# sea-sky-web/Vision-based-Spatio-Temporal-Analysis

Measured on AMD Instinct MI355X. Metric: multi-cam frames/sec (7-cam→480×1440 BEV), higher is better.
Workload: dtype f32; 1 GPU; 7-cam 1080x1920 -> resnet50(stride-8 features)+proj C=64 -> IPM warp -> mean -> 480x1440 BEV (BASELINE configs[1]); cameras=7, cameras_per_gpu=7, channels=64, bev_memory_format=NCHW, parallelism=frame-sharded x1 (no collective)

## Files before the change

### vision-based-spatio-temporal-analysis_amd/csrc/bev_conv_x6.hip

```cpp
#include <hip/hip_runtime.h>
#include <stdint.h>

#include <type_traits>

#include "../../include/bev_mi355x.h"
#include "bev_act.h"

namespace {

typedef __bf16 bf16x8 __attribute__((ext_vector_type(8)));
typedef __bf16 bf16x4 __attribute__((ext_vector_type(4)));
typedef float f32x16 __attribute__((ext_vector_type(16)));
typedef float f32x4 __attribute__((ext_vector_type(4)));
typedef unsigned u32x4 __attribute__((ext_vector_type(4)));
typedef unsigned u32x2 __attribute__((ext_vector_type(2)));

#ifndef X6S_T_EPI
#define X6S_T_EPI 0
#endif
#ifndef X6S_ABLATE
#define X6S_ABLATE 0
#endif
constexpr int XBK = 16;
constexpr int XROW = 24;

__device__ __attribute__((aligned(16))) float g_xzero4[4] = {0.f, 0.f, 0.f, 0.f};

__host__ __device__ inline int64_t kpad_x(int K) { return (K + XBK - 1) / XBK * XBK; }
__host__ __device__ inline int64_t copad_x(int Co) { return (Co + 127) / 128 * 128; }

__device__ __forceinline__ void split3(float v, __bf16 &h, __bf16 &m, __bf16 &l) {
    h = (__bf16)v;
    const float r = v - (float)h;
    m = (__bf16)r;
    l = (__bf16)(r - (float)m);
}

__host__ __device__ inline int64_t frag_index(int n, int k, int p, int64_t S) {
    return (((int64_t)(n >> 5) * S + (k >> 4)) * 3 + p) * 512 + (((k >> 3) & 1) * 32 + (n & 31)) * 8 + (k & 7);
}

__global__ void k_pack_x6(const float *__restrict__ w, int Co, int Ci, int KH, int KW, int64_t Kp, int64_t Cop,
                          __bf16 *__restrict__ out) {
    const int64_t t = (int64_t)blockIdx.x * blockDim.x + threadIdx.x;
    if (t >= Kp * Cop) return;
    const int n = (int)(t / Kp);
    const int k = (int)(t % Kp);
    const int K = Ci * KH * KW;
    float v = 0.0f;
    if (n < Co && k < K) {
        const int ci = k % Ci, r = k / Ci, kx = r % KW, ky = r / KW;
        v = w[(((int64_t)n * Ci + ci) * KH + ky) * KW + kx];
    }
    __bf16 h, m, l;
    split3(v, h, m, l);
    const int64_t S = Kp / XBK;
    out[frag_index(n, k, 0, S)] = h;
    out[frag_index(n, k, 1, S)] = m;
    out[frag_index(n, k, 2, S)] = l;
}

struct ConvX {
    const float *__restrict__ x;
    const __bf16 *__restrict__ wp;
    const float *__restrict__ bias;
    const float *__restrict__ res;
    float *__restrict__ y;
    int N, H, W, Ci, Co, KH, KW, stride, pad, dil, Ho, Wo, act, ldy, Kp;
    int64_t M;
    const float *__restrict__ x2;
    int Ci2, H2, W2, stride2;
    const __bf16 *__restrict__ xs;
    __bf16 *__restrict__ ys;
    int64_t xps, yps;
    const __bf16 *__restrict__ wp2;
    const float *__restrict__ bias2;
    int Co2, act2;
    int nta = 0;
    const __bf16 *__restrict__ wp3 = nullptr;
    const float *__restrict__ bias3 = nullptr;
    __bf16 *__restrict__ ys3 = nullptr;
    float *__restrict__ y3 = nullptr;
    int Co3 = 0, act3 = 0;
};

__device__ __forceinline__ float act_x(float t, int act) {
    if (act == 2) return silu_hw(t);
    if (act == 1) return t > 0.0f ? t : 0.0f;
    return t;
}

template <int TN>
__host__ __device__ constexpr int x6_epi_bytes() { return 4 * 32 * (TN * 32 + 4) * 4; }

template <int TM, int TN>
__device__ __forceinline__ void x6_epilogue(const ConvX &a, float *lds, const f32x16 (&acc)[TM][TN], int wave,
                                            int lane, int wn, int wm, int64_t m0, int n0) {
    const int r32 = lane & 31, h = lane >> 5;
    constexpr int WC = TN * 32, ER = WC + 4;
    constexpr int C4 = WC / 4, RPI = 64 / C4, NQ = 32 / RPI;
    float *E = lds + wave * (32 * ER);
    const int c4 = lane % C4, rq = lane / C4;
    const int n = n0 + wn * WC + c4 * 4;
    const bool nvec = ((a.Co & 3) == 0) && ((a.ldy & 3) == 0) && (n + 3 < a.Co);
    float4 rv[NQ];
    auto res_load = [&](int i) {
        const int64_t mb = m0 + wm * TM * 32 + i * 32;
#pragma unroll
        for (int q = 0; q < NQ; ++q) {
            const int64_t m = mb + rq + RPI * q;
            rv[q] = make_float4(0.f, 0.f, 0.f, 0.f);
            if (a.res && m < a.M && nvec) rv[q] = *(const float4 *)(a.res + m * a.Co + n);
        }
    };
    res_load(0);
    __syncthreads();
    float4 bv = make_float4(0.f, 0.f, 0.f, 0.f);
    if (a.bias) {
        if (nvec) bv = *(const float4 *)(a.bias + n);
        else {
            bv.x = n < a.Co ? a.bias[n] : 0.f;
            bv.y = n + 1 < a.Co ? a.bias[n + 1] : 0.f;
            bv.z = n + 2 < a.Co ? a.bias[n + 2] : 0.f;
            bv.w = n + 3 < a.Co ? a.bias[n + 3] : 0.f;
        }
    }
#pragma unroll
    for (int i = 0; i < TM; ++i) {
#pragma unroll
        for (int j = 0; j < TN; ++j)
#pragma unroll
            for (int r = 0; r < 16; ++r) E[((r & 3) + 8 * (r >> 2) + 4 * h) * ER + j * 32 + r32] = acc[i][j][r];
        const int64_t mbase = m0 + wm * TM * 32 + i * 32;
        if (i > 0) res_load(i);
#pragma unroll
        for (int q = 0; q < NQ; ++q) {
            const int row = rq + RPI * q;
            const int64_t m = mbase + row;
            if (m >= a.M) continue;
            const float4 v = *(const float4 *)(E + row * ER + c4 * 4);
            float o[4] = {v.x + bv.x, v.y + bv.y, v.z + bv.z, v.w + bv.w};
            if (a.ys) {
                if (a.res) {
                    const float4 rr = rv[q];
                    o[0] += rr.x, o[1] += rr.y, o[2] += rr.z, o[3] += rr.w;
                }
                bf16x4 hv, mv, lv;
#pragma unroll
                for (int u = 0; u < 4; ++u) {
                    __bf16 h_, m_, l_;
                    split3(act_x(o[u], a.act), h_, m_, l_);
                    hv[u] = h_, mv[u] = m_, lv[u] = l_;
                }
                __bf16 *yp = a.ys + m * a.Co + n;
                if (n < a.Co) {
                    *(bf16x4 *)yp = hv;
                    *(bf16x4 *)(yp + a.yps) = mv;
                    *(bf16x4 *)(yp + 2 * a.yps) = lv;
                }
                continue;
            }
            float *yp = a.y + m * a.ldy + n;
            if (nvec) {
                if (a.res) {
                    o[0] += rv[q].x;
                    o[1] += rv[q].y;
                    o[2] += rv[q].z;
                    o[3] += rv[q].w;
                }
#pragma unroll
                for (int u = 0; u < 4; ++u) o[u] = act_x(o[u], a.act);
                *(float4 *)yp = make_float4(o[0], o[1], o[2], o[3]);
            } else {
#pragma unroll
                for (int u = 0; u < 4; ++u) {
                    if (n + u >= a.Co) break;
                    float t = o[u];
                    if (a.res) t += a.res[m * a.Co + n + u];
                    yp[u] = act_x(t, a.act);
                }
            }
        }
    }
}

template <int WM, int WN, int TM, int TN, bool DUAL>
__global__ __launch_bounds__(256, 2) void k_conv_x6(ConvX a) {
    constexpr int BM = WM * TM * 32, BN = WN * TN * 32;
    constexpr int APL = BM * XROW, BPL = BN * XROW;
    constexpr int STAGE = 3 * (APL + BPL);
    constexpr int AQ = BM / 64;
    constexpr int PB = ((BN * 6) % 256 == 0) ? 16 : 8;
    constexpr int PPR = 96 / PB;
    constexpr int BQ = BN * PPR / 256;
    static_assert(BN * PPR % 256 == 0, "B pieces per thread");
    typedef typename std::conditional<PB == 16, u32x4, u32x2>::type bpiece;
    constexpr int EPIB = x6_epi_bytes<TN>();
    constexpr int LDSB = (2 * STAGE * 2 > EPIB) ? 2 * STAGE * 2 : EPIB;
    static_assert(BM % 64 == 0, "A staging rows");
    __shared__ __attribute__((aligned(16))) unsigned char lds_raw[LDSB];
    __bf16 *lds = (__bf16 *)lds_raw;

    const int tid = threadIdx.x;
    const int lane = tid & 63, wave = __builtin_amdgcn_readfirstlane(tid >> 6);
    const int wm = wave / WN, wn = wave % WN;
    const int n_tiles = (a.Co + BN - 1) / BN;
    unsigned bid = blockIdx.x;
    {
        const unsigned nb = gridDim.x, q = nb / 8, r = nb % 8, xc = bid % 8;
        bid = (xc < r ? xc * (q + 1) : r * (q + 1) + (xc - r) * q) + bid / 8;
    }
    const int64_t m0 = (int64_t)(bid / n_tiles) * BM;
    const int n0 = (bid % n_tiles) * BN;

    const int aq = tid & 3;
    int64_t pb[AQ], p2[AQ];
    int iy0[AQ], ix0[AQ];
    bool rok[AQ];
#pragma unroll
    for (int q = 0; q < AQ; ++q) {
        const int64_t m = m0 + (tid >> 2) + 64 * q;
        rok[q] = m < a.M;
        const int64_t mm = rok[q] ? m : 0;
        const int ox = (int)(mm % a.Wo);
        const int64_t t = mm / a.Wo;
        const int oy = (int)(t % a.Ho);
        const int64_t n = t / a.Ho;
        if (DUAL) {
            pb[q] = mm * a.Ci + 4 * aq;
            p2[q] = ((n * a.H2 + (int64_t)oy * a.stride2) * a.W2 + (int64_t)ox * a.stride2) * a.Ci2 + 4 * aq;
            iy0[q] = ix0[q] = 0;
        } else {
            pb[q] = n * a.H * a.W * a.Ci + 4 * aq;
            p2[q] = 0;
            iy0[q] = oy * a.stride - a.pad;
            ix0[q] = ox * a.stride - a.pad;
        }
    }
    const int64_t bstep = 3 * 512;
    const __bf16 *brow[BQ];
    int bdst[BQ];
#pragma unroll
    for (int i = 0; i < BQ; ++i) {
        const int pc = tid + 256 * i;
        const int row = pc / PPR, byte = (pc % PPR) * PB;
        const int pl = byte / 32, hk = (byte % 32) / 16, sub = (byte % 16) / 2;
        brow[i] = a.wp + frag_index(n0 + row, 8 * hk, pl, a.Kp / XBK) + sub;
        bdst[i] = pl * BPL + row * XROW + 8 * hk + sub;
    }
    f32x16 acc[TM][TN];
#pragma unroll
    for (int i = 0; i < TM; ++i)
#pragma unroll
        for (int j = 0; j < TN; ++j) acc[i][j] = (f32x16){0};

    f32x4 va0[AQ], va1[AQ];
    bpiece vb0[BQ], vb1[BQ];
    int ky = 0, kx = 0, ci0 = 0, k0 = 0;
    int64_t kb = 0;
#define X6_GLOAD(VA, VB)                                                                                   \
    do {                                                                                                   \
        if (DUAL) {                                                                                        \
            const bool first = k0 < a.Ci;                                                                  \
            const float *src = first ? a.x + k0 : a.x2 + (k0 - a.Ci);                                      \
            _Pragma("unroll") for (int q = 0; q < AQ; ++q) VA[q] =                                         \
                *(const f32x4 *)(rok[q] ? src + (first ? pb[q] : p2[q]) : g_xzero4);                      \
// ... 23 lines not shown
        __bf16 *Bs = As + 3 * APL;                                                                         \
        _Pragma("unroll") for (int q = 0; q < AQ; ++q) {                                                   \
            bf16x4 hv, mv, lv;                                                                             \
            _Pragma("unroll") for (int e = 0; e < 4; ++e) {                                                \
                __bf16 h_, m_, l_;                                                                         \
                split3(VA[q][e], h_, m_, l_);                                                              \
                hv[e] = h_;                                                                                \
                mv[e] = m_;                                                                                \
                lv[e] = l_;                                                                                \
            }                                                                                              \
            __bf16 *d = As + ((tid >> 2) + 64 * q) * XROW + 4 * aq;                                        \
            *(bf16x4 *)d = hv;                                                                             \
            *(bf16x4 *)(d + APL) = mv;                                                                     \
            *(bf16x4 *)(d + 2 * APL) = lv;                                                                 \
        }                                                                                                  \
        _Pragma("unroll") for (int i = 0; i < BQ; ++i) *(bpiece *)(Bs + bdst[i]) = VB[i];                \
    } while (0)
    const int r32 = lane & 31, h = lane >> 5;
#define X6_MFMA(BUF)                                                                                       \
    do {                                                                                                   \
        const __bf16 *As = lds + (BUF) * STAGE;                                                            \
        const __bf16 *Bs = As + 3 * APL;                                                                   \
        bf16x8 fa[TM][3], fb[TN][3];                                                                       \
        _Pragma("unroll") for (int i = 0; i < TM; ++i)                                                     \
            _Pragma("unroll") for (int p = 0; p < 3; ++p)                                                  \
                fa[i][p] = *(const bf16x8 *)(As + p * APL + (wm * TM * 32 + i * 32 + r32) * XROW + 8 * h); \
        _Pragma("unroll") for (int j = 0; j < TN; ++j)                                                     \
            _Pragma("unroll") for (int p = 0; p < 3; ++p)                                                  \
                fb[j][p] = *(const bf16x8 *)(Bs + p * BPL + (wn * TN * 32 + j * 32 + r32) * XROW + 8 * h); \
        _Pragma("unroll") for (int i = 0; i < TM; ++i)                                                     \
            _Pragma("unroll") for (int j = 0; j < TN; ++j) {                                               \
                acc[i][j] = __builtin_amdgcn_mfma_f32_32x32x16_bf16(fa[i][0], fb[j][0], acc[i][j], 0, 0, 0); \
                acc[i][j] = __builtin_amdgcn_mfma_f32_32x32x16_bf16(fa[i][0], fb[j][1], acc[i][j], 0, 0, 0); \
                acc[i][j] = __builtin_amdgcn_mfma_f32_32x32x16_bf16(fa[i][1], fb[j][0], acc[i][j], 0, 0, 0); \
                acc[i][j] = __builtin_amdgcn_mfma_f32_32x32x16_bf16(fa[i][0], fb[j][2], acc[i][j], 0, 0, 0); \
                acc[i][j] = __builtin_amdgcn_mfma_f32_32x32x16_bf16(fa[i][2], fb[j][0], acc[i][j], 0, 0, 0); \
                acc[i][j] = __builtin_amdgcn_mfma_f32_32x32x16_bf16(fa[i][1], fb[j][1], acc[i][j], 0, 0, 0); \
            }                                                                                              \
    } while (0)

    const int nk = a.Kp / XBK;
    X6_GLOAD(va0, vb0);
    if (nk > 1) X6_GLOAD(va1, vb1);
    X6_SWRITE(0, va0, vb0);
    __syncthreads();
    int ks = 0;
    for (; ks + 3 < nk; ks += 2) {
        X6_GLOAD(va0, vb0);
        X6_MFMA(0);
        X6_SWRITE(1, va1, vb1);
        __syncthreads();
        X6_GLOAD(va1, vb1);
        X6_MFMA(1);
        X6_SWRITE(0, va0, vb0);
        __syncthreads();
    }
    if (ks + 2 < nk) {
        X6_GLOAD(va0, vb0);
        X6_MFMA(0);
        X6_SWRITE(1, va1, vb1);
        __syncthreads();
        X6_MFMA(1);
        X6_SWRITE(0, va0, vb0);
        __syncthreads();
        X6_MFMA(0);
    } else if (ks + 1 < nk) {
        X6_MFMA(0);
        X6_SWRITE(1, va1, vb1);
        __syncthreads();
        X6_MFMA(1);
    } else {
        X6_MFMA(0);
    }
#undef X6_MFMA
#undef X6_SWRITE
#undef X6_GLOAD
    x6_epilogue<TM, TN>(a, (float *)lds_raw, acc, wave, lane, wn, wm, m0, n0);
}

__device__ __forceinline__ __amdgpu_buffer_rsrc_t x6_rsrc(const void *p, int64_t bytes) {
    return __builtin_amdgcn_make_buffer_rsrc(const_cast<void *>(p), 0, (int)(uint32_t)bytes, 0x00020000);
}

template <int WM, int WN, int TM, int TN, int X2S = 0>
__device__ __forceinline__ void x6_chain_epilogue(const ConvX &a, unsigned char *lds_raw, const f32x16 (&acc)[TM][TN],
                                                  int wave, int lane, int wm, int wn, int64_t m0) {
    constexpr int BM = WM * TM * 32, BN = WN * TN * 32, HR = BN + 8, HPL = BM * HR;
    constexpr int NB = BM / 32, WPB = 4 / NB;
    static_assert(NB * WPB == 4, "chain epilogue: 4 waves over the 32-row bands");
    __bf16 *H = (__bf16 *)lds_raw;
    const int r32 = lane & 31, hh = lane >> 5;
    const int band = (wave % NB) * 32, part = wave / NB;
    const int64_t rows = (a.M - m0 < BM) ? a.M - m0 : BM;
    const int64_t base = m0 * a.Co2;
    const __amdgpu_buffer_rsrc_t rr = x6_rsrc(a.res ? a.res + base : a.y + base, rows * a.Co2 * 4);
    const int vo = ((band + 4 * hh) * a.Co2 + r32) * 4;
    const int nch = a.Co2 / 64 / WPB;
    float rvn[2][16];
    auto res_load = [&](int c0) {
        if (!a.res) return;
#pragma unroll
        for (int j = 0; j < 2; ++j)
#pragma unroll
            for (int r = 0; r < 16; ++r)
                rvn[j][r] = __builtin_bit_cast(
                    float, __builtin_amdgcn_raw_buffer_load_b32(rr, vo + ((r & 3) + 8 * (r >> 2)) * a.Co2 * 4,
                                                                (c0 + 32 * j) * 4, 0));
    };
    res_load(64 * part * nch);
    __syncthreads();
#pragma unroll
    for (int i = 0; i < TM; ++i)
#pragma unroll
        for (int j = 0; j < TN; ++j) {
            const int col = wn * TN * 32 + j * 32 + r32;
            const float bj = a.bias ? a.bias[col] : 0.0f;
#pragma unroll
            for (int r = 0; r < 16; ++r) {
                __bf16 h_, m_, l_;
                split3(act_x(acc[i][j][r] + bj, a.act), h_, m_, l_);
                const int row = wm * TM * 32 + i * 32 + (r & 3) + 8 * (r >> 2) + 4 * hh;
                H[row * HR + col] = h_;
                H[HPL + row * HR + col] = m_;
                H[2 * HPL + row * HR + col] = l_;
            }
        }
    __syncthreads();
    constexpr int S2 = BN / 16;
    constexpr int ST = S2 + X2S;
    bf16x8 fx[X2S > 0 ? X2S : 1][3];
    if constexpr (X2S > 0) {
        int64_t m = m0 + band + r32;
        const bool ok = m < a.M;
        m = ok ? m : 0;
        const int ox = (int)(m % a.Wo);
        const int64_t q = m / a.Wo;
        const int oy = (int)(q % a.Ho);
        const int64_t n = q / a.Ho;
        const float *xp = a.x2 + ((n * a.H2 + (int64_t)oy * a.stride2) * a.W2 + (int64_t)ox * a.stride2) * a.Ci2 + 8 * hh;
#pragma unroll
        for (int t = 0; t < X2S; ++t) {
            f32x4 v0 = ok ? *(const f32x4 *)(xp + 16 * t) : (f32x4){0.f, 0.f, 0.f, 0.f};
            f32x4 v1 = ok ? *(const f32x4 *)(xp + 16 * t + 4) : (f32x4){0.f, 0.f, 0.f, 0.f};
#pragma unroll
            for (int e = 0; e < 8; ++e) {
                __bf16 h_, m_, l_;
                split3(e < 4 ? v0[e] : v1[e - 4], h_, m_, l_);
                fx[t][0][e] = h_, fx[t][1][e] = m_, fx[t][2][e] = l_;
            }
        }
    }
    const __bf16 *ap = H + (band + r32) * HR + 8 * hh;
    const __amdgpu_buffer_rsrc_t ry = x6_rsrc(a.y + base, rows * a.Co2 * 4);
    const __amdgpu_buffer_rsrc_t rw = x6_rsrc(a.wp2, copad_x(a.Co2) / 32 * (int64_t)ST * 3072);
    const int vl = lane * 16;
    for (int nc = part * nch; nc < (part + 1) * nch; ++nc) {
        const int c0 = 64 * nc;
        float rv[2][16];
#pragma unroll
        for (int j = 0; j < 2; ++j)
#pragma unroll
            for (int r = 0; r < 16; ++r) rv[j][r] = rvn[j][r];
        if (nc + 1 < (part + 1) * nch) res_load(c0 + 64);
        f32x16 acc2[2] = {(f32x16){0}, (f32x16){0}};
#pragma unroll
        for (int t = 0; t < ST; ++t) {
            bf16x8 fa[3], fb[2][3];
#pragma unroll
            for (int p = 0; p < 3; ++p) {
                if constexpr (X2S > 0) fa[p] = t < S2 ? *(const bf16x8 *)(ap + p * HPL + 16 * (t < S2 ? t : 0))
                                                      : fx[t >= S2 ? t - S2 : 0][p];
                else fa[p] = *(const bf16x8 *)(ap + p * HPL + 16 * t);
            }
#pragma unroll
            for (int j = 0; j < 2; ++j)
#pragma unroll
                for (int p = 0; p < 3; ++p)
                    fb[j][p] = __builtin_bit_cast(
                        bf16x8, __builtin_amdgcn_raw_buffer_load_b128(rw, vl, (((c0 >> 5) + j) * ST + t) * 3072 + p * 1024, 0));
#pragma unroll
            for (int j = 0; j < 2; ++j) {
                acc2[j] = __builtin_amdgcn_mfma_f32_32x32x16_bf16(fa[0], fb[j][0], acc2[j], 0, 0, 0);
                acc2[j] = __builtin_amdgcn_mfma_f32_32x32x16_bf16(fa[0], fb[j][1], acc2[j], 0, 0, 0);
                acc2[j] = __builtin_amdgcn_mfma_f32_32x32x16_bf16(fa[1], fb[j][0], acc2[j], 0, 0, 0);
                acc2[j] = __builtin_amdgcn_mfma_f32_32x32x16_bf16(fa[0], fb[j][2], acc2[j], 0, 0, 0);
                acc2[j] = __builtin_amdgcn_mfma_f32_32x32x16_bf16(fa[2], fb[j][0], acc2[j], 0, 0, 0);
                acc2[j] = __builtin_amdgcn_mfma_f32_32x32x16_bf16(fa[1], fb[j][1], acc2[j], 0, 0, 0);
            }
        }
#pragma unroll
        for (int j = 0; j < 2; ++j) {
            const float bj = a.bias2 ? a.bias2[c0 + 32 * j + r32] : 0.0f;
#pragma unroll
            for (int r = 0; r < 16; ++r) {
                float o = acc2[j][r] + bj;
                if (a.res) o += rv[j][r];
                o = act_x(o, a.act2);
                __builtin_amdgcn_raw_buffer_store_b32(__builtin_bit_cast(unsigned, o), ry,
                                                      vo + ((r & 3) + 8 * (r >> 2)) * a.Co2 * 4, (c0 + 32 * j) * 4, 0);
            }
        }
    }
}

template <int WM, int WN, int TM, int TN, int X2S = 0, int NT3 = 0>
__device__ __forceinline__ void x6_chain_epilogue_t(const ConvX &a, unsigned char *lds_raw,
                                                    const f32x16 (&acc)[TM][TN], int wave, int lane, int wm, int wn,
                                                    int64_t m0) {
    constexpr int BM = WM * TM * 32, BN = WN * TN * 32, HR = BN + 8, HPL = BM * HR;
    constexpr int NB = BM / 32, WPB = 4 / NB;
    static_assert(NB * WPB == 4, "chain epilogue: 4 waves over the 32-row bands");
    static_assert(NT3 == 0 || WPB == 1, "the fused next conv needs all of a band's Co2 chunks in one wave");
    __bf16 *H = (__bf16 *)lds_raw;
    const int r32 = lane & 31, hh = lane >> 5;
    const int band = (wave % NB) * 32, part = wave / NB;
    const int64_t rows = (a.M - m0 < BM) ? a.M - m0 : BM;
    const int64_t base = m0 * a.Co2;
    const __amdgpu_buffer_rsrc_t rr = x6_rsrc(a.res ? a.res + base : a.y + base, rows * a.Co2 * 4);
    const int vrow = (band + r32) * a.Co2 * 4 + 16 * hh;
    const int nch = a.Co2 / 64 / WPB;
    f32x4 rvn[2][4];
    auto res_load = [&](int c0) {
        if (!a.res) return;
#pragma unroll
        for (int j = 0; j < 2; ++j)
#pragma unroll
            for (int g = 0; g < 4; ++g)
                rvn[j][g] = __builtin_bit_cast(f32x4, __builtin_amdgcn_raw_buffer_load_b128(rr, vrow + 32 * g,
                                                                                           (c0 + 32 * j) * 4, 0));
    };
    res_load(64 * part * nch);
    __syncthreads();
#pragma unroll
    for (int i = 0; i < TM; ++i)
#pragma unroll
        for (int j = 0; j < TN; ++j) {
            const int col = wn * TN * 32 + j * 32 + r32;
            const float bj = a.bias ? a.bias[col] : 0.0f;
#pragma unroll
            for (int r = 0; r < 16; ++r) {
                __bf16 h_, m_, l_;
                split3(act_x(acc[i][j][r] + bj, a.act), h_, m_, l_);
                const int row = wm * TM * 32 + i * 32 + (r & 3) + 8 * (r >> 2) + 4 * hh;
                H[row * HR + col] = h_;
                H[HPL + row * HR + col] = m_;
                H[2 * HPL + row * HR + col] = l_;
            }
        }
    __syncthreads();
    constexpr int S2 = BN / 16;
    constexpr int ST = S2 + X2S;
    bf16x8 fx[X2S > 0 ? X2S : 1][3];
    if constexpr (X2S > 0) {
        int64_t m = m0 + band + r32;
        const bool ok = m < a.M;
        m = ok ? m : 0;
        const int ox = (int)(m % a.Wo);
        const int64_t q = m / a.Wo;
        const int oy = (int)(q % a.Ho);
        const int64_t n = q / a.Ho;
        const float *xp = a.x2 + ((n * a.H2 + (int64_t)oy * a.stride2) * a.W2 + (int64_t)ox * a.stride2) * a.Ci2 + 8 * hh;
#pragma unroll
        for (int t = 0; t < X2S; ++t) {
            f32x4 v0 = ok ? *(const f32x4 *)(xp + 16 * t) : (f32x4){0.f, 0.f, 0.f, 0.f};
            f32x4 v1 = ok ? *(const f32x4 *)(xp + 16 * t + 4) : (f32x4){0.f, 0.f, 0.f, 0.f};
#pragma unroll
            for (int e = 0; e < 8; ++e) {
                __bf16 h_, m_, l_;
                split3(e < 4 ? v0[e] : v1[e - 4], h_, m_, l_);
                fx[t][0][e] = h_, fx[t][1][e] = m_, fx[t][2][e] = l_;
            }
        }
    }
    const __bf16 *ap = H + (band + r32) * HR + 8 * hh;
    const __amdgpu_buffer_rsrc_t ry = x6_rsrc(a.y + base, rows * a.Co2 * 4);
    const __amdgpu_buffer_rsrc_t rw = x6_rsrc(a.wp2, copad_x(a.Co2) / 32 * (int64_t)ST * 3072);
    const int vl = lane * 16;
    constexpr int N3 = NT3 > 0 ? NT3 : 1;
    const int S3 = a.Co2 / 16;
    const __amdgpu_buffer_rsrc_t rw3 = x6_rsrc(NT3 > 0 ? a.wp3 : a.wp2, NT3 > 0 ? copad_x(a.Co3) / 32 * (int64_t)S3 * 3072 : 0);
    f32x16 acc3[N3];
#pragma unroll
    for (int q = 0; q < N3; ++q) acc3[q] = (f32x16){0};
    for (int nc = part * nch; nc < (part + 1) * nch; ++nc) {
        const int c0 = 64 * nc;
// ... 53 lines not shown
                        return (unsigned)__builtin_bit_cast(unsigned short, x0) |
                               ((unsigned)__builtin_bit_cast(unsigned short, x1) << 16);
                    };
                    ys[j][g][0][0] = pk(hv[0], hv[1]), ys[j][g][0][1] = pk(hv[2], hv[3]);
                    ys[j][g][1][0] = pk(mv[0], mv[1]), ys[j][g][1][1] = pk(mv[2], mv[3]);
                    ys[j][g][2][0] = pk(lv[0], lv[1]), ys[j][g][2][1] = pk(lv[2], lv[3]);
                }
            }
        if constexpr (NT3 > 0) {
#pragma unroll
            for (int j = 0; j < 2; ++j)
#pragma unroll
                for (int sl = 0; sl < 2; ++sl) {
                    bf16x8 fy[3];
#pragma unroll
                    for (int p = 0; p < 3; ++p) {
                        const unsigned k0 = ys[j][2 * sl][p][0], k1 = ys[j][2 * sl][p][1];
                        const unsigned q0 = ys[j][2 * sl + 1][p][0], q1 = ys[j][2 * sl + 1][p][1];
                        const unsigned s0 = hh ? k0 : q0, s1 = hh ? k1 : q1;
                        const unsigned r0 = (unsigned)__shfl_xor((int)s0, 32), r1 = (unsigned)__shfl_xor((int)s1, 32);
                        const u32x4 f = hh ? (u32x4){r0, r1, q0, q1} : (u32x4){k0, k1, r0, r1};
                        fy[p] = __builtin_bit_cast(bf16x8, f);
                    }
                    const int ks = (c0 + 32 * j + 16 * sl) >> 4;
#pragma unroll
                    for (int q = 0; q < NT3; ++q) {
                        bf16x8 fw3[3];
#pragma unroll
                        for (int p = 0; p < 3; ++p)
                            fw3[p] = __builtin_bit_cast(
                                bf16x8, __builtin_amdgcn_raw_buffer_load_b128(rw3, vl, (q * S3 + ks) * 3072 + p * 1024, 0));
                        acc3[q] = __builtin_amdgcn_mfma_f32_32x32x16_bf16(fw3[0], fy[0], acc3[q], 0, 0, 0);
                        acc3[q] = __builtin_amdgcn_mfma_f32_32x32x16_bf16(fw3[1], fy[0], acc3[q], 0, 0, 0);
                        acc3[q] = __builtin_amdgcn_mfma_f32_32x32x16_bf16(fw3[0], fy[1], acc3[q], 0, 0, 0);
                        acc3[q] = __builtin_amdgcn_mfma_f32_32x32x16_bf16(fw3[2], fy[0], acc3[q], 0, 0, 0);
                        acc3[q] = __builtin_amdgcn_mfma_f32_32x32x16_bf16(fw3[0], fy[2], acc3[q], 0, 0, 0);
                        acc3[q] = __builtin_amdgcn_mfma_f32_32x32x16_bf16(fw3[1], fy[1], acc3[q], 0, 0, 0);
                    }
                }
        }
    }
    if constexpr (NT3 > 0) {
        const int64_t prow = m0 + band + r32;
        if (prow < a.M) {
#pragma unroll
            for (int q = 0; q < NT3; ++q)
#pragma unroll
                for (int g = 0; g < 4; ++g) {
                    const int c = 32 * q + 8 * g + 4 * hh;
                    const f32x4 bv = a.bias3 ? *(const f32x4 *)(a.bias3 + c) : (f32x4){0.f, 0.f, 0.f, 0.f};
                    f32x4 o;
#pragma unroll
                    for (int u = 0; u < 4; ++u) o[u] = act_x(acc3[q][4 * g + u] + bv[u], a.act3);
                    if (a.ys3) {
                        bf16x4 hv, mv, lv;
#pragma unroll
                        for (int u = 0; u < 4; ++u) {
                            __bf16 h_, m_, l_;
                            split3(o[u], h_, m_, l_);
                            hv[u] = h_, mv[u] = m_, lv[u] = l_;
                        }
                        __bf16 *yp = a.ys3 + prow * a.Co3 + c;
                        const int64_t pl = a.M * a.Co3;
                        *(bf16x4 *)yp = hv;
                        *(bf16x4 *)(yp + pl) = mv;
                        *(bf16x4 *)(yp + 2 * pl) = lv;
                    } else {
                        *(f32x4 *)(a.y3 + prow * a.Co3 + c) = o;
                    }
                }
        }
    }
}

constexpr int YBK = 32;
constexpr int YROW = 40;

template <int WM, int WN, int TM, int TN, bool DUAL, int CHAIN = 0, bool NT = false>
__global__ __launch_bounds__(256, 2) void k_conv_x6b(ConvX a) {
    constexpr int BM = WM * TM * 32, BN = WN * TN * 32;
    constexpr int APL = BM * YROW;
    constexpr int STAGE = 3 * APL;
    constexpr int AQ = BM / 32;
    constexpr int EPIB = CHAIN ? 3 * BM * (BN + 8) * 2 : x6_epi_bytes<TN>();
    constexpr int LDSB = (2 * STAGE * 2 > EPIB) ? 2 * STAGE * 2 : EPIB;
    __shared__ __attribute__((aligned(16))) unsigned char lds_raw[LDSB];
    __bf16 *lds = (__bf16 *)lds_raw;

    const int tid = threadIdx.x;
    const int lane = tid & 63, wave = __builtin_amdgcn_readfirstlane(tid >> 6);
    const int wm = wave / WN, wn = wave % WN;
    const int n_tiles = (a.Co + BN - 1) / BN;
    unsigned bid = blockIdx.x;
    {
        const unsigned nb = gridDim.x, q = nb / 8, r = nb % 8, xc = bid % 8;
        bid = (xc < r ? xc * (q + 1) : r * (q + 1) + (xc - r) * q) + bid / 8;
    }
    const int64_t m0 = (int64_t)(bid / n_tiles) * BM;
    const int n0 = (bid % n_tiles) * BN;

    const int aq = tid & 7;
    int64_t pb[AQ], p2[AQ];
    int iy0[AQ], ix0[AQ];
    bool rok[AQ];
#pragma unroll
    for (int q = 0; q < AQ; ++q) {
        const int64_t m = m0 + (tid >> 3) + 32 * q;
        rok[q] = m < a.M;
        const int64_t mm = rok[q] ? m : 0;
        const int ox = (int)(mm % a.Wo);
        const int64_t t = mm / a.Wo;
        const int oy = (int)(t % a.Ho);
        const int64_t n = t / a.Ho;
        if (DUAL) {
            pb[q] = mm * a.Ci + 4 * aq;
            p2[q] = ((n * a.H2 + (int64_t)oy * a.stride2) * a.W2 + (int64_t)ox * a.stride2) * a.Ci2 + 4 * aq;
            iy0[q] = ix0[q] = 0;
        } else {
            pb[q] = n * a.H * a.W * a.Ci + 4 * aq;
            p2[q] = 0;
            iy0[q] = oy * a.stride - a.pad;
            ix0[q] = ox * a.stride - a.pad;
        }
    }
    const int64_t S = a.Kp / XBK;
    const __bf16 *wb = a.wp + ((int64_t)((n0 + wn * TN * 32) >> 5) * S) * 1536 + lane * 8;
    const int nslice = a.Kp / XBK;

    f32x16 acc[TM][TN];
#pragma unroll
    for (int i = 0; i < TM; ++i)
#pragma unroll
        for (int j = 0; j < TN; ++j) acc[i][j] = (f32x16){0};

    f32x4 va0[AQ], va1[AQ];
    bf16x8 bs0[TN][3], bs1[TN][3];
    int ky = 0, kx = 0, ci0 = 0, k0 = 0;
#define X6B_GLOAD(VA)                                                                                      \
    do {                                                                                                   \
        if (DUAL) {                                                                                        \
            const bool first = k0 < a.Ci;                                                                  \
            const float *src = first ? a.x + k0 : a.x2 + (k0 - a.Ci);                                      \
            _Pragma("unroll") for (int q = 0; q < AQ; ++q) VA[q] =                                         \
                *(const f32x4 *)(rok[q] ? src + (first ? pb[q] : p2[q]) : g_xzero4);                      \
            k0 += YBK;                                                                                     \
        } else {                                                                                           \
            const int dy = ky * a.dil, dx = kx * a.dil;                                                    \
            _Pragma("unroll") for (int q = 0; q < AQ; ++q) {                                               \
                const int iy = iy0[q] + dy, ix = ix0[q] + dx;                                              \
                const bool in = rok[q] && (unsigned)iy < (unsigned)a.H && (unsigned)ix < (unsigned)a.W;    \
                const f32x4 *ap_ = (const f32x4 *)(in ? a.x + pb[q] + ((int64_t)iy * a.W + ix) * a.Ci + ci0 : g_xzero4); \
                if (NT) VA[q] = __builtin_nontemporal_load(ap_);                                          \
                else VA[q] = *ap_;                                                                        \
            }                                                                                              \
            ci0 += YBK;                                                                                    \
            if (ci0 == a.Ci) {                                                                             \
                ci0 = 0;                                                                                   \
                if (++kx == a.KW) {                                                                        \
                    kx = 0;                                                                                \
                    ++ky;                                                                                  \
                }                                                                                          \
            }                                                                                              \
        }                                                                                                  \
    } while (0)
#define X6B_SWRITE(BUF, VA)                                                                                \
    do {                                                                                                   \
        __bf16 *As = lds + (BUF) * STAGE;                                                                  \
// ... 27 lines not shown
            _Pragma("unroll") for (int p = 0; p < 3; ++p)                                                  \
                fa[i][p] = *(const bf16x8 *)(AS + p * APL + (wm * TM * 32 + i * 32 + r32) * YROW + 16 * (KK) + 8 * h); \
        _Pragma("unroll") for (int i = 0; i < TM; ++i)                                                     \
            _Pragma("unroll") for (int j = 0; j < TN; ++j) {                                               \
                acc[i][j] = __builtin_amdgcn_mfma_f32_32x32x16_bf16(fa[i][0], BC[j][0], acc[i][j], 0, 0, 0); \
                acc[i][j] = __builtin_amdgcn_mfma_f32_32x32x16_bf16(fa[i][0], BC[j][1], acc[i][j], 0, 0, 0); \
                acc[i][j] = __builtin_amdgcn_mfma_f32_32x32x16_bf16(fa[i][1], BC[j][0], acc[i][j], 0, 0, 0); \
                acc[i][j] = __builtin_amdgcn_mfma_f32_32x32x16_bf16(fa[i][0], BC[j][2], acc[i][j], 0, 0, 0); \
                acc[i][j] = __builtin_amdgcn_mfma_f32_32x32x16_bf16(fa[i][2], BC[j][0], acc[i][j], 0, 0, 0); \
                acc[i][j] = __builtin_amdgcn_mfma_f32_32x32x16_bf16(fa[i][1], BC[j][1], acc[i][j], 0, 0, 0); \
            }                                                                                              \
    } while (0)
#define X6B_MFMA(BUF, KS)                                                                                  \
    do {                                                                                                   \
        const __bf16 *As = lds + (BUF) * STAGE;                                                            \
        X6B_SLICE(As, 0, bs0);                                                                             \
        X6B_BLOAD(bs0, 2 * (KS) + 2);                                                                      \
        X6B_SLICE(As, 1, bs1);                                                                             \
    } while (0)

    const int nk = a.Kp / YBK;
    X6B_BLOAD(bs0, 0);
    X6B_GLOAD(va0);
    if (nk > 1) X6B_GLOAD(va1);
    X6B_SWRITE(0, va0);
    __syncthreads();
    int ks = 0;
    for (; ks + 3 < nk; ks += 2) {
        X6B_BLOAD(bs1, 2 * ks + 1);
        X6B_GLOAD(va0);
        X6B_MFMA(0, ks);
        X6B_SWRITE(1, va1);
        __syncthreads();
        X6B_BLOAD(bs1, 2 * ks + 3);
        X6B_GLOAD(va1);
        X6B_MFMA(1, ks + 1);
        X6B_SWRITE(0, va0);
        __syncthreads();
    }
    if (ks + 2 < nk) {
        X6B_BLOAD(bs1, 2 * ks + 1);
        X6B_GLOAD(va0);
        X6B_MFMA(0, ks);
        X6B_SWRITE(1, va1);
        __syncthreads();
        X6B_BLOAD(bs1, 2 * ks + 3);
        X6B_MFMA(1, ks + 1);
        X6B_SWRITE(0, va0);
        __syncthreads();
        X6B_BLOAD(bs1, 2 * ks + 5);
        X6B_MFMA(0, ks + 2);
    } else if (ks + 1 < nk) {
        X6B_BLOAD(bs1, 2 * ks + 1);
        X6B_MFMA(0, ks);
        X6B_SWRITE(1, va1);
        __syncthreads();
        X6B_BLOAD(bs1, 2 * ks + 3);
        X6B_MFMA(1, ks + 1);
    } else {
        X6B_BLOAD(bs1, 2 * ks + 1);
        X6B_MFMA(0, ks);
    }
#undef X6B_MFMA
#undef X6B_SLICE
#undef X6B_BLOAD
#undef X6B_SWRITE
#undef X6B_GLOAD
    if constexpr (CHAIN > 0) {
        if (X6S_ABLATE & 1) {
            float s_ = 0.0f;
#pragma unroll
            for (int i = 0; i < TM; ++i)
#pragma unroll
                for (int j = 0; j < TN; ++j) s_ += acc[i][j][0] + acc[i][j][15];
            if (m0 + tid < a.M) a.y[(m0 + tid) * a.Co2] = s_;
            return;
        }
        x6_chain_epilogue<WM, WN, TM, TN, CHAIN == 2 ? 4 : 0>(a, lds_raw, acc, wave, lane, wm, wn, m0);
        return;
    }
    x6_epilogue<TM, TN>(a, (float *)lds_raw, acc, wave, lane, wn, wm, m0, n0);
}

__device__ __forceinline__ unsigned lds_addr(const void *p) {
    return (unsigned)(uintptr_t)(const __attribute__((address_space(3))) void *)p;
}

__device__ __forceinline__ void dma16(const void *src, unsigned dst_any) {
    const unsigned dst = (unsigned)__builtin_amdgcn_readfirstlane((int)dst_any);
    unsigned keep;
    asm volatile(
        "s_mov_b32 %0, m0\n\ts_mov_b32 m0, %2\n\ts_nop 0\n\t"
        "global_load_lds_dwordx4 %1, off\n\ts_mov_b32 m0, %0"
        : "=&s"(keep)
        : "v"(src), "s"(dst)
        : "memory");
}

template <int WM, int WN, int TM, int TN, int CHAIN = 0, bool BLDS = (CHAIN > 0), int NT3 = 0>
__global__ __launch_bounds__(256, CHAIN ? 2 : 3) void k_conv_x6s(ConvX a) {
    constexpr int BM = WM * TM * 32, BN = WN * TN * 32;
    constexpr int APL = BM * 32;
    constexpr int BST = BLDS ? BN / 32 * 6 * 512 : 0;
    constexpr int STAGE = 3 * APL + BST;
    constexpr int RW = BM / 4;
    constexpr int RG = RW / 16;
    constexpr int BPW = BLDS ? BN / 32 * 6 / 4 : 0;
    constexpr int EPIB = CHAIN ? 3 * BM * (BN + 8) * 2 : x6_epi_bytes<TN>();
    constexpr int LDSB = (2 * STAGE * 2 > EPIB) ? 2 * STAGE * 2 : EPIB;
    static_assert(RW % 16 == 0, "whole DMA groups per wave");
    static_assert(!BLDS || (BN / 32 * 6) % 4 == 0, "whole B pieces per wave");
    __shared__ __attribute__((aligned(16))) unsigned char lds_raw[LDSB];
    const __bf16 *lds = (const __bf16 *)lds_raw;

    const int tid = threadIdx.x;
    const int lane = tid & 63, wave = __builtin_amdgcn_readfirstlane(tid >> 6);
    const int wm = wave / WN, wn = wave % WN;
    const int n_tiles = (a.Co + BN - 1) / BN;
    unsigned bid = blockIdx.x;
    {
        const unsigned nb = gridDim.x, q = nb / 8, r = nb % 8, xc = bid % 8;
        bid = (xc < r ? xc * (q + 1) : r * (q + 1) + (xc - r) * q) + bid / 8;
    }
    const int64_t m0 = (int64_t)(bid / n_tiles) * BM;
    const int n0 = (bid % n_tiles) * BN;

    int64_t abase[RG];
    int aiy[RG], aix[RG];
    bool aok[RG];
#pragma unroll
    for (int g = 0; g < RG; ++g) {
        const int row = wave * RW + 16 * g + (lane >> 2);
        const int lc = (lane & 3) ^ ((row >> 2) & 3);
        const int64_t m = m0 + row;
        aok[g] = m < a.M;
        const int64_t mm = aok[g] ? m : 0;
        const int ox = (int)(mm % a.Wo);
        const int64_t t = mm / a.Wo;
        const int oy = (int)(t % a.Ho);
        const int64_t n = t / a.Ho;
        aiy[g] = oy * a.stride - a.pad;
        aix[g] = ox * a.stride - a.pad;
        abase[g] = ((n * a.H + aiy[g]) * a.W + aix[g]) * a.Ci + 8 * lc;
    }
    const unsigned lbase = (unsigned)__builtin_amdgcn_readfirstlane((int)lds_addr(lds_raw));
    const int S = a.Kp / XBK;
    int ky = 0, kx = 0, ci0 = 0, kstep = 0;
    const __bf16 *bsrc = a.wp + (int64_t)(n0 >> 5) * S * 1536 + lane * 8;
    auto issue = [&](int buf) {
        if (X6S_ABLATE & 4) return;
        if constexpr (BLDS) {
            const unsigned db = lbase + (unsigned)(buf * STAGE * 2 + 3 * APL * 2);
#pragma unroll
            for (int i = 0; i < BPW; ++i) {
                const int q = wave + 4 * i, cbl = q / 6, r = q % 6;
                dma16(bsrc + ((int64_t)cbl * S + 2 * kstep + r / 3) * 1536 + (r % 3) * 512,
                      db + (unsigned)(q * 1024));
            }
            ++kstep;
        }
        const int64_t toff = ((int64_t)ky * a.dil * a.W + kx * a.dil) * a.Ci + ci0;
        const unsigned d0 = lbase + (unsigned)(buf * STAGE * 2) + (unsigned)(wave * RW * 64);
#pragma unroll
        for (int g = 0; g < RG; ++g) {
            const int iy = aiy[g] + ky * a.dil, ix = aix[g] + kx * a.dil;
            const bool in = aok[g] && (unsigned)iy < (unsigned)a.H && (unsigned)ix < (unsigned)a.W;
            const __bf16 *src = a.xs + abase[g] + toff;
#pragma unroll
            for (int p = 0; p < 3; ++p)
                dma16(in ? (const void *)(src + p * a.xps) : (const void *)g_xzero4,
                      d0 + (unsigned)(p * APL * 2 + g * 1024));
        }
        ci0 += YBK;
        if (ci0 == a.Ci) {
            ci0 = 0;
            if (++kx == a.KW) {
                kx = 0;
                ++ky;
            }
        }
    };

    const __amdgpu_buffer_rsrc_t rw = __builtin_amdgcn_make_buffer_rsrc(
        const_cast<__bf16 *>(a.wp), 0, (int)(uint32_t)(copad_x(a.Co) / 32 * (int64_t)S * 3072), 0x00020000);
    const int cb0 = (n0 + wn * TN * 32) >> 5;
    const int vl = lane * 16;
    bf16x8 bs0[TN][3], bs1[TN][3];
#define X6S_BLOAD(BS, G)                                                                                   \
    do {                                                                                                   \
        const int g_ = (G) < S ? (G) : S - 1;                                                              \
        _Pragma("unroll") for (int j = 0; j < TN; ++j)                                                     \
// ... 778 lines not shown
```

Baseline: 133.2 frames/s.

## Stage chained-conv weights in LDS via async DMA with double buffering

The fused chain epilogue of the second 1x1 conv now streams its weight fragments into a double-buffered LDS region using global_load_lds DMA, instead of issuing per-wave buffer loads straight into registers. The A fragments are hoisted into registers once, and the output channels are processed in 32-wide groups with residual and bias prefetch for the next group. Activation functions are dispatched at compile time through templates rather than branched per element. In exchange the kernel needs more LDS, hand-written vmcnt waits and barriers, and more registers, which may lower occupancy.

```diff
diff --git a/vision-based-spatio-temporal-analysis_amd/csrc/bev_conv_x6.hip b/vision-based-spatio-temporal-analysis_amd/csrc/bev_conv_x6.hip
--- a/vision-based-spatio-temporal-analysis_amd/csrc/bev_conv_x6.hip
+++ b/vision-based-spatio-temporal-analysis_amd/csrc/bev_conv_x6.hip
@@ -90,6 +90,20 @@
     return t;
 }
 
+template <int ACT>
+__device__ __forceinline__ float act_c(float t) {
+    if constexpr (ACT == 2) return silu_hw(t);
+    else if constexpr (ACT == 1) return t > 0.0f ? t : 0.0f;
+    else return t;
+}
+
+template <class F>
+__device__ __forceinline__ void act_dispatch(int act, F &&f) {
+    if (act == 2) f(std::integral_constant<int, 2>{});
+    else if (act == 1) f(std::integral_constant<int, 1>{});
+    else f(std::integral_constant<int, 0>{});
+}
+
 template <int TN>
 __host__ __device__ constexpr int x6_epi_bytes() { return 4 * 32 * (TN * 32 + 4) * 4; }
 
@@ -125,63 +139,66 @@
             bv.w = n + 3 < a.Co ? a.bias[n + 3] : 0.f;
         }
     }
-#pragma unroll
-    for (int i = 0; i < TM; ++i) {
-#pragma unroll
-        for (int j = 0; j < TN; ++j)
-#pragma unroll
-            for (int r = 0; r < 16; ++r) E[((r & 3) + 8 * (r >> 2) + 4 * h) * ER + j * 32 + r32] = acc[i][j][r];
-        const int64_t mbase = m0 + wm * TM * 32 + i * 32;
-        if (i > 0) res_load(i);
-#pragma unroll
-        for (int q = 0; q < NQ; ++q) {
-            const int row = rq + RPI * q;
-            const int64_t m = mbase + row;
-            if (m >= a.M) continue;
-            const float4 v = *(const float4 *)(E + row * ER + c4 * 4);
-            float o[4] = {v.x + bv.x, v.y + bv.y, v.z + bv.z, v.w + bv.w};
-            if (a.ys) {
-                if (a.res) {
-                    const float4 rr = rv[q];
-                    o[0] += rr.x, o[1] += rr.y, o[2] += rr.z, o[3] += rr.w;
+    act_dispatch(a.act, [&](auto ac) {
+        constexpr int ACT = decltype(ac)::value;
+#pragma unroll
+        for (int i = 0; i < TM; ++i) {
+#pragma unroll
+            for (int j = 0; j < TN; ++j)
+#pragma unroll
+                for (int r = 0; r < 16; ++r) E[((r & 3) + 8 * (r >> 2) + 4 * h) * ER + j * 32 + r32] = acc[i][j][r];
+            const int64_t mbase = m0 + wm * TM * 32 + i * 32;
+            if (i > 0) res_load(i);
+#pragma unroll
+            for (int q = 0; q < NQ; ++q) {
+                const int row = rq + RPI * q;
+                const int64_t m = mbase + row;
+                if (m >= a.M) continue;
+                const float4 v = *(const float4 *)(E + row * ER + c4 * 4);
+                float o[4] = {v.x + bv.x, v.y + bv.y, v.z + bv.z, v.w + bv.w};
+                if (a.ys) {
+                    if (a.res) {
+                        const float4 rr = rv[q];
+                        o[0] += rr.x, o[1] += rr.y, o[2] += rr.z, o[3] += rr.w;
+                    }
+                    bf16x4 hv, mv, lv;
+#pragma unroll
+                    for (int u = 0; u < 4; ++u) {
+                        __bf16 h_, m_, l_;
+                        split3(act_c<ACT>(o[u]), h_, m_, l_);
+                        hv[u] = h_, mv[u] = m_, lv[u] = l_;
+                    }
+                    __bf16 *yp = a.ys + m * a.Co + n;
+                    if (n < a.Co) {
+                        *(bf16x4 *)yp = hv;
+                        *(bf16x4 *)(yp + a.yps) = mv;
+                        *(bf16x4 *)(yp + 2 * a.yps) = lv;
+                    }
+                    continue;
                 }
-                bf16x4 hv, mv, lv;
-#pragma unroll
-                for (int u = 0; u < 4; ++u) {
-                    __bf16 h_, m_, l_;
-                    split3(act_x(o[u], a.act), h_, m_, l_);
-                    hv[u] = h_, mv[u] = m_, lv[u] = l_;
-                }
-                __bf16 *yp = a.ys + m * a.Co + n;
-                if (n < a.Co) {
-                    *(bf16x4 *)yp = hv;
-                    *(bf16x4 *)(yp + a.yps) = mv;
-                    *(bf16x4 *)(yp + 2 * a.yps) = lv;
-                }
-                continue;
-            }
-            float *yp = a.y + m * a.ldy + n;
-            if (nvec) {
-                if (a.res) {
-                    o[0] += rv[q].x;
-                    o[1] += rv[q].y;
-                    o[2] += rv[q].z;
-                    o[3] += rv[q].w;
-                }
-#pragma unroll
-                for (int u = 0; u < 4; ++u) o[u] = act_x(o[u], a.act);
-                *(float4 *)yp = make_float4(o[0], o[1], o[2], o[3]);
-            } else {
-#pragma unroll
-                for (int u = 0; u < 4; ++u) {
-                    if (n + u >= a.Co) break;
-                    float t = o[u];
-                    if (a.res) t += a.res[m * a.Co + n + u];
-                    yp[u] = act_x(t, a.act);
+                float *yp = a.y + m * a.ldy + n;
+                if (nvec) {
+                    if (a.res) {
+                        o[0] += rv[q].x;
+                        o[1] += rv[q].y;
+                        o[2] += rv[q].z;
+                        o[3] += rv[q].w;
+                    }
+#pragma unroll
+                    for (int u = 0; u < 4; ++u) o[u] = act_c<ACT>(o[u]);
+                    *(float4 *)yp = make_float4(o[0], o[1], o[2], o[3]);
+                } else {
+#pragma unroll
+                    for (int u = 0; u < 4; ++u) {
+                        if (n + u >= a.Co) break;
+                        float t = o[u];
+                        if (a.res) t += a.res[m * a.Co + n + u];
+                        yp[u] = act_c<ACT>(t);
+                    }
                 }
             }
         }
-    }
+    });
 }
 
 template <int WM, int WN, int TM, int TN, bool DUAL>
@@ -371,53 +388,104 @@
     return __builtin_amdgcn_make_buffer_rsrc(const_cast<void *>(p), 0, (int)(uint32_t)bytes, 0x00020000);
 }
 
+__device__ __forceinline__ unsigned lds_addr(const void *p) {
+    return (unsigned)(uintptr_t)(const __attribute__((address_space(3))) void *)p;
+}
+
+__device__ __forceinline__ void dma16(const void *src, unsigned dst_any) {
+    const unsigned dst = (unsigned)__builtin_amdgcn_readfirstlane((int)dst_any);
+    unsigned keep;
+    asm volatile(
+        "s_mov_b32 %0, m0\n\ts_mov_b32 m0, %2\n\ts_nop 0\n\t"
+        "global_load_lds_dwordx4 %1, off\n\ts_mov_b32 m0, %0"
+        : "=&s"(keep)
+        : "v"(src), "s"(dst)
+        : "memory");
+}
+
+template <int N>
+__device__ __forceinline__ void x6_wait_barrier() {
+    static_assert(N >= 0 && N < 64, "vmcnt is a 6-bit counter");
+    asm volatile("s_waitcnt vmcnt(%0) lgkmcnt(0)\n\ts_barrier" ::"n"(N) : "memory");
+}
+
+template <int BM, int BN>
+__host__ __device__ constexpr int x6_chain_lds_bytes() { return 3 * BM * (BN + 8) * 2 + (4 / (BM / 32)) * 12288; }
+
 template <int WM, int WN, int TM, int TN, int X2S = 0>
 __device__ __forceinline__ void x6_chain_epilogue(const ConvX &a, unsigned char *lds_raw, const f32x16 (&acc)[TM][TN],
                                                   int wave, int lane, int wm, int wn, int64_t m0) {
     constexpr int BM = WM * TM * 32, BN = WN * TN * 32, HR = BN + 8, HPL = BM * HR;
     constexpr int NB = BM / 32, WPB = 4 / NB;
     static_assert(NB * WPB == 4, "chain epilogue: 4 waves over the 32-row bands");
+    constexpr int S2 = BN / 16;
+    constexpr int ST = S2 + X2S;
+    constexpr int U = ST / 4;
+    static_assert(ST % 4 == 0, "chain epilogue: whole 4-slice steps");
+    constexpr int HB = 3 * HPL * 2;
+    constexpr int PW = WPB * 3;
+    static_assert(HB % 1024 == 0, "W3 stage 0 starts on a fragment boundary");
     __bf16 *H = (__bf16 *)lds_raw;
     const int r32 = lane & 31, hh = lane >> 5;
     const int band = (wave % NB) * 32, part = wave / NB;
     const int64_t rows = (a.M - m0 < BM) ? a.M - m0 : BM;
     const int64_t base = m0 * a.Co2;
-    const __amdgpu_buffer_rsrc_t rr = x6_rsrc(a.res ? a.res + base : a.y + base, rows * a.Co2 * 4);
+    const float *resp = a.res ? a.res + base : a.y + base;
+    const float *biasp = a.bias2 ? a.bias2 : a.y;
+    const int64_t resb = rows * a.Co2 * 4, biasb = a.bias2 ? (int64_t)a.Co2 * 4 : 0;
     const int vo = ((band + 4 * hh) * a.Co2 + r32) * 4;
-    const int nch = a.Co2 / 64 / WPB;
-    float rvn[2][16];
-    auto res_load = [&](int c0) {
-        if (!a.res) return;
-#pragma unroll
-        for (int j = 0; j < 2; ++j)
+    const int NG = a.Co2 / (32 * WPB);
+    auto res_load = [&](auto hr, int c0, float(&rv)[17], bool live) {
+        const __amdgpu_buffer_rsrc_t rr = x6_rsrc(resp, live ? resb : 0), rb = x6_rsrc(biasp, live ? biasb : 0);
+        rv[16] = __builtin_bit_cast(float, __builtin_amdgcn_raw_buffer_load_b32(rb, r32 * 4, c0 * 4, 0));
+        if constexpr (decltype(hr)::value) {
 #pragma unroll
             for (int r = 0; r < 16; ++r)
-                rvn[j][r] = __builtin_bit_cast(
-                    float, __builtin_amdgcn_raw_buffer_load_b32(rr, vo + ((r & 3) + 8 * (r >> 2)) * a.Co2 * 4,
-                                                                (c0 + 32 * j) * 4, 0));
+                rv[r] = __builtin_bit_cast(float, __builtin_amdgcn_raw_buffer_load_b32(
+                                                      rr, vo + ((r & 3) + 8 * (r >> 2)) * a.Co2 * 4, c0 * 4, 0));
+        }
     };
-    res_load(64 * part * nch);
+    const unsigned lbase = (unsigned)__builtin_amdgcn_readfirstlane((int)lds_addr(lds_raw));
+    const __bf16 *wsrc = a.wp2 + lane * 8;
+    auto issue_w3 = [&](int g, int u, unsigned sbo) {
+#pragma unroll
+        for (int i = 0; i < PW; ++i) {
+            const int q = wave + 4 * i, cbl = q / 12, r = q % 12;
+            dma16(wsrc + (((int64_t)(g * WPB + cbl) * ST + 4 * u) * 3 + r) * 512, lbase + sbo + (unsigned)(q * 1024));
+        }
+    };
+    float rv[2][17];
+    if (a.res) res_load(std::true_type{}, 32 * part, rv[0], true);
+    else res_load(std::false_type{}, 32 * part, rv[0], true);
     __syncthreads();
-#pragma unroll
-    for (int i = 0; i < TM; ++i)
-#pragma unroll
-        for (int j = 0; j < TN; ++j) {
-            const int col = wn * TN * 32 + j * 32 + r32;
-            const float bj = a.bias ? a.bias[col] : 0.0f;
-#pragma unroll
-            for (int r = 0; r < 16; ++r) {
-                __bf16 h_, m_, l_;
-                split3(act_x(acc[i][j][r] + bj, a.act), h_, m_, l_);
-                const int row = wm * TM * 32 + i * 32 + (r & 3) + 8 * (r >> 2) + 4 * hh;
-                H[row * HR + col] = h_;
-                H[HPL + row * HR + col] = m_;
-                H[2 * HPL + row * HR + col] = l_;
+    issue_w3(0, 0, HB);
+    act_dispatch(a.act, [&](auto ac) {
+#pragma unroll
+        for (int i = 0; i < TM; ++i)
+#pragma unroll
+            for (int j = 0; j < TN; ++j) {
+                const int col = wn * TN * 32 + j * 32 + r32;
+                const float bj = a.bias ? a.bias[col] : 0.0f;
+#pragma unroll
+                for (int r = 0; r < 16; ++r) {
+                    __bf16 h_, m_, l_;
+                    split3(act_c<decltype(ac)::value>(acc[i][j][r] + bj), h_, m_, l_);
+                    const int row = wm * TM * 32 + i * 32 + (r & 3) + 8 * (r >> 2) + 4 * hh;
+                    H[row * HR + col] = h_;
+                    H[HPL + row * HR + col] = m_;
+                    H[2 * HPL + row * HR + col] = l_;
+                }
             }
-        }
+    });
     __syncthreads();
-    constexpr int S2 = BN / 16;
-    constexpr int ST = S2 + X2S;
-    bf16x8 fx[X2S > 0 ? X2S : 1][3];
+    bf16x8 fa[ST][3];
+    {
+        const __bf16 *ap = H + (band + r32) * HR + 8 * hh;
+#pragma unroll
+        for (int t = 0; t < S2; ++t)
+#pragma unroll
+            for (int p = 0; p < 3; ++p) fa[t][p] = *(const bf16x8 *)(ap + p * HPL + 16 * t);
+    }
     if constexpr (X2S > 0) {
         int64_t m = m0 + band + r32;
         const bool ok = m < a.M;
@@ -435,61 +503,71 @@
             for (int e = 0; e < 8; ++e) {
                 __bf16 h_, m_, l_;
                 split3(e < 4 ? v0[e] : v1[e - 4], h_, m_, l_);
-                fx[t][0][e] = h_, fx[t][1][e] = m_, fx[t][2][e] = l_;
+                fa[S2 + t][0][e] = h_, fa[S2 + t][1][e] = m_, fa[S2 + t][2][e] = l_;
             }
         }
     }
-    const __bf16 *ap = H + (band + r32) * HR + 8 * hh;
+    asm volatile("s_waitcnt vmcnt(0) lgkmcnt(0)" ::: "memory");
     const __amdgpu_buffer_rsrc_t ry = x6_rsrc(a.y + base, rows * a.Co2 * 4);
-    const __amdgpu_buffer_rsrc_t rw = x6_rsrc(a.wp2, copad_x(a.Co2) / 32 * (int64_t)ST * 3072);
-    const int vl = lane * 16;
-    for (int nc = part * nch; nc < (part + 1) * nch; ++nc) {
-        const int c0 = 64 * nc;
-        float rv[2][16];
-#pragma unroll
-        for (int j = 0; j < 2; ++j)
-#pragma unroll
-            for (int r = 0; r < 16; ++r) rv[j][r] = rvn[j][r];
-        if (nc + 1 < (part + 1) * nch) res_load(c0 + 64);
-        f32x16 acc2[2] = {(f32x16){0}, (f32x16){0}};
-#pragma unroll
-        for (int t = 0; t < ST; ++t) {
-            bf16x8 fa[3], fb[2][3];
-#pragma unroll
-            for (int p = 0; p < 3; ++p) {
-                if constexpr (X2S > 0) fa[p] = t < S2 ? *(const bf16x8 *)(ap + p * HPL + 16 * (t < S2 ? t : 0))
-                                                      : fx[t >= S2 ? t - S2 : 0][p];
-                else fa[p] = *(const bf16x8 *)(ap + p * HPL + 16 * t);
+    auto block = [&](auto hr, auto a2, int g, float(&rc)[17], float(&rn)[17]) {
+        constexpr bool HAS_RES = decltype(hr)::value;
+        constexpr int R = HAS_RES ? 17 : 1;
+        const bool more = g + 1 < NG;
+        const int c0 = 32 * (g * WPB + part);
+        f32x16 acc2 = (f32x16){0};
+#pragma unroll
+        for (int u = 0; u < U; ++u) {
+            if constexpr (U == 1) x6_wait_barrier<R + 16>();
+            else if (u == 0) x6_wait_barrier<16>();
+            else if (u == 1) x6_wait_barrier<R>();
+            else x6_wait_barrier<0>();
+            const unsigned sbo = ((g * U + u) & 1) ? 0u : (unsigned)HB;
+            if (u + 1 < U) issue_w3(g, u + 1, (unsigned)HB - sbo);
+            else if (more) issue_w3(g + 1, 0, (unsigned)HB - sbo);
+            if (u == 0) {
+                res_load(hr, c0 + 32 * WPB, rn, more);
+                asm volatile("" ::: "memory");
             }
-#pragma unroll
-            for (int j = 0; j < 2; ++j)
-#pragma unroll
-                for (int p = 0; p < 3; ++p)
-                    fb[j][p] = __builtin_bit_cast(
-                        bf16x8, __builtin_amdgcn_raw_buffer_load_b128(rw, vl, (((c0 >> 5) + j) * ST + t) * 3072 + p * 1024, 0));
-#pragma unroll
-            for (int j = 0; j < 2; ++j) {
-                acc2[j] = __builtin_amdgcn_mfma_f32_32x32x16_bf16(fa[0], fb[j][0], acc2[j], 0, 0, 0);
-                acc2[j] = __builtin_amdgcn_mfma_f32_32x32x16_bf16(fa[0], fb[j][1], acc2[j], 0, 0, 0);
-                acc2[j] = __builtin_amdgcn_mfma_f32_32x32x16_bf16(fa[1], fb[j][0], acc2[j], 0, 0, 0);
-                acc2[j] = __builtin_amdgcn_mfma_f32_32x32x16_bf16(fa[0], fb[j][2], acc2[j], 0, 0, 0);
-                acc2[j] = __builtin_amdgcn_mfma_f32_32x32x16_bf16(fa[2], fb[j][0], acc2[j], 0, 0, 0);
-                acc2[j] = __builtin_amdgcn_mfma_f32_32x32x16_bf16(fa[1], fb[j][1], acc2[j], 0, 0, 0);
+            const __bf16 *Bs = (const __bf16 *)(lds_raw + sbo) + part * (12 * 512) + lane * 8;
+#pragma unroll
+            for (int sl = 0; sl < 4; ++sl) {
+                const int t = 4 * u + sl;
+                bf16x8 fb[3];
+#pragma unroll
+                for (int p = 0; p < 3; ++p) fb[p] = *(const bf16x8 *)(Bs + (sl * 3 + p) * 512);
+                acc2 = __builtin_amdgcn_mfma_f32_32x32x16_bf16(fa[t][0], fb[0], acc2, 0, 0, 0);
+                acc2 = __builtin_amdgcn_mfma_f32_32x32x16_bf16(fa[t][0], fb[1], acc2, 0, 0, 0);
+                acc2 = __builtin_amdgcn_mfma_f32_32x32x16_bf16(fa[t][1], fb[0], acc2, 0, 0, 0);
+                acc2 = __builtin_amdgcn_mfma_f32_32x32x16_bf16(fa[t][0], fb[2], acc2, 0, 0, 0);
+                acc2 = __builtin_amdgcn_mfma_f32_32x32x16_bf16(fa[t][2], fb[0], acc2, 0, 0, 0);
+                acc2 = __builtin_amdgcn_mfma_f32_32x32x16_bf16(fa[t][1], fb[1], acc2, 0, 0, 0);
             }
         }
-#pragma unroll
-        for (int j = 0; j < 2; ++j) {
-            const float bj = a.bias2 ? a.bias2[c0 + 32 * j + r32] : 0.0f;
-#pragma unroll
-            for (int r = 0; r < 16; ++r) {
-                float o = acc2[j][r] + bj;
-                if (a.res) o += rv[j][r];
-                o = act_x(o, a.act2);
-                __builtin_amdgcn_raw_buffer_store_b32(__builtin_bit_cast(unsigned, o), ry,
-                                                      vo + ((r & 3) + 8 * (r >> 2)) * a.Co2 * 4, (c0 + 32 * j) * 4, 0);
-            }
-        }
-    }
+        const float bj = rc[16];
+#pragma unroll
+        for (int r = 0; r < 16; ++r) {
+            float o = acc2[r] + bj;
+            if constexpr (HAS_RES) o += rc[r];
+            o = act_c<decltype(a2)::value>(o);
+            __builtin_amdgcn_raw_buffer_store_b32(__builtin_bit_cast(unsigned, o), ry,
+                                                  vo + ((r & 3) + 8 * (r >> 2)) * a.Co2 * 4, c0 * 4, 0);
+        }
+    };
+    auto run = [&](auto hr, auto a2) {
+        asm volatile("" ::"v"(rv[0][16]));
+        if constexpr (decltype(hr)::value) {
+#pragma unroll
+            for (int r = 0; r < 16; ++r) asm volatile("" ::"v"(rv[0][r]));
+        }
+        for (int g = 0; g < NG; g += 2) {
+            block(hr, a2, g, rv[0], rv[1]);
+            if (g + 1 < NG) block(hr, a2, g + 1, rv[1], rv[0]);
+        }
+    };
+    act_dispatch(a.act2, [&](auto a2) {
+        if (a.res) run(std::true_type{}, a2);
+        else run(std::false_type{}, a2);
+    });
 }
 
 template <int WM, int WN, int TM, int TN, int X2S = 0, int NT3 = 0>
@@ -709,7 +787,7 @@
     constexpr int APL = BM * YROW;
     constexpr int STAGE = 3 * APL;
     constexpr int AQ = BM / 32;
-    constexpr int EPIB = CHAIN ? 3 * BM * (BN + 8) * 2 : x6_epi_bytes<TN>();
+    constexpr int EPIB = CHAIN ? x6_chain_lds_bytes<BM, BN>() : x6_epi_bytes<TN>();
     constexpr int LDSB = (2 * STAGE * 2 > EPIB) ? 2 * STAGE * 2 : EPIB;
     __shared__ __attribute__((aligned(16))) unsigned char lds_raw[LDSB];
     __bf16 *lds = (__bf16 *)lds_raw;
@@ -903,21 +981,6 @@
     x6_epilogue<TM, TN>(a, (float *)lds_raw, acc, wave, lane, wn, wm, m0, n0);
 }
 
-__device__ __forceinline__ unsigned lds_addr(const void *p) {
-    return (unsigned)(uintptr_t)(const __attribute__((address_space(3))) void *)p;
-}
-
-__device__ __forceinline__ void dma16(const void *src, unsigned dst_any) {
-    const unsigned dst = (unsigned)__builtin_amdgcn_readfirstlane((int)dst_any);
-    unsigned keep;
-    asm volatile(
-        "s_mov_b32 %0, m0\n\ts_mov_b32 m0, %2\n\ts_nop 0\n\t"
-        "global_load_lds_dwordx4 %1, off\n\ts_mov_b32 m0, %0"
-        : "=&s"(keep)
-        : "v"(src), "s"(dst)
-        : "memory");
-}
-
 template <int WM, int WN, int TM, int TN, int CHAIN = 0, bool BLDS = (CHAIN > 0), int NT3 = 0>
 __global__ __launch_bounds__(256, CHAIN ? 2 : 3) void k_conv_x6s(ConvX a) {
     constexpr int BM = WM * TM * 32, BN = WN * TN * 32;
@@ -927,7 +990,7 @@
     constexpr int RW = BM / 4;
     constexpr int RG = RW / 16;
     constexpr int BPW = BLDS ? BN / 32 * 6 / 4 : 0;
-    constexpr int EPIB = CHAIN ? 3 * BM * (BN + 8) * 2 : x6_epi_bytes<TN>();
+    constexpr int EPIB = CHAIN ? x6_chain_lds_bytes<BM, BN>() : x6_epi_bytes<TN>();
     constexpr int LDSB = (2 * STAGE * 2 > EPIB) ? 2 * STAGE * 2 : EPIB;
     static_assert(RW % 16 == 0, "whole DMA groups per wave");
     static_assert(!BLDS || (BN / 32 * 6) % 4 == 0, "whole B pieces per wave");
```

Result: faster. 138.3 frames/s, median of 6 (+3.8%).
